# stablecabal/gyre

Hardware: AMD Instinct MI355X
Metric: SD1.5 512px 50-step images/sec (node) (higher is better)
Workload: dtype bf16

## Files before the change

gyre_amd/build.py:

```python
from __future__ import annotations

import os
import subprocess
import sys
from concurrent.futures import ThreadPoolExecutor

HERE = os.path.dirname(os.path.abspath(__file__))
CSRC = os.path.join(HERE, "csrc")
LIB = os.path.join(HERE, "libgyre_hip.so")
LIB_F16 = os.path.join(HERE, "libgyre_hip_f16.so")
SOURCES = ["kernels_elem.hip", "kernels_gemm.hip", "kernels_gemm4s.hip", "kernels_gemm_ar.hip", "kernels_gemm_sm.hip", "kernels_conv_out.hip", "kernels_attn.hip", "kernels_xattn.hip", "kernels_tome.hip", "kernels_bwd.hip", "kernels_t2i.hip", "model.hip", "model_vjp.hip", "model_t2i.hip"]
HEADERS = ["common.h", "kernels.h", "gemm_shared.h", "model_impl.h", os.path.join("..", "..", "include", "gyre_hip.h")]
FLAGS = ["--offload-arch=gfx950", "-O3", "-std=c++17", "-fPIC", "-mcode-object-version=5",
         "-Wno-unused-result", "-fno-gpu-rdc",
         "-mllvm", "-pragma-unroll-threshold=1000000"]


PER_FILE_FLAGS = {"kernels_attn.hip": ["-mllvm", "-amdgpu-mfma-vgpr-form=1"]}

RESOURCE_FILES = ("kernels_attn.hip", "kernels_gemm.hip", "kernels_gemm4s.hip", "kernels_gemm_ar.hip", "kernels_gemm_sm.hip")
SCRATCH_ALLOWED = ("k_attn3ILi80E", "k_gemm4s")
RESOURCES_JSON = os.path.join(HERE, "build", "kernel_resources.json")


def _hipcc() -> str:
    for c in (os.environ.get("HIPCC"), "/opt/rocm/bin/hipcc", "hipcc"):
        if c and (os.path.isabs(c) and os.path.exists(c) or not os.path.isabs(c)):
            return c
    raise RuntimeError("hipcc not found")


def _stale(out: str, deps) -> bool:
    if not os.path.exists(out):
        return True
    t = os.path.getmtime(out)
# ... 95 lines not shown
```

gyre_amd/csrc/kernels.h:

```cpp
#pragma once
#include "common.h"

int launch_nchw_to_nhwc(hipStream_t st, const void* x, int dtype, int B, int C, int HW, int Cpad, bf16_t* y);
int launch_add_nchw_into_nhwc(hipStream_t st, const void* r, int dtype, int B, int C, int HW, int Cpad, bf16_t* y);
int launch_ctx_to_bf16(hipStream_t st, const void* x, int dtype, size_t n, bf16_t* y);
int launch_dup_batch(hipStream_t st, const void* src, void* dst, size_t outer, size_t inner_bytes);
int launch_add_f32(hipStream_t st, float* y, const float* x, size_t n);
int launch_verify_hints(hipStream_t st, const int64_t* t, int B, int check_t, const void* x, size_t bytes_per_half, int check_pairs, int* flag);
int launch_timestep_embedding(hipStream_t st, const int64_t* t, int B, int dim, int flip, float shift, float* out);
int launch_rowvec_linear(hipStream_t st, float* x, int B, int K, const bf16_t* W, const float* bias, int N,
                         int act_in_silu, float* out, int ldo);
int launch_timestep_linear(hipStream_t st, const int64_t* t, int B, int dim, int flip, float shift, float* emb_scratch,
                           const bf16_t* W, const float* bias, int N, float* out, int ldo);

struct GnParams {
    const bf16_t* x; const bf16_t* x2; int C1;
    int B, HW, C, G;
    const float* gamma; const float* beta; float eps; int silu;
    float* partial;
    float* scale_shift;
    int nchunks;
    bf16_t* y;
    float* mean_rstd = nullptr;
    const float* cs_x = nullptr; int cs_x_chunks = 0;
// ... 15 lines not shown
    GEMM_DBG_NO_GN_FOLD       = 0x1000,
    GEMM_DBG_NO_XATTN         = 0x2000,
    GEMM_DBG_NO_GEGLU_4S      = 0x4000,
    GEMM_DBG_LN_STATS_PASS    = 0x8000,
    GEMM_DBG_GEGLU_NO_LN_FOLD = 0x10000,
    GEMM_DBG_GN_STATS_PASS    = 0x20000,
    GEMM_DBG_NO_128x160       = 0x40000,
    GEMM_DBG_NO_CS_128x160    = 0x100000,
    GEMM_DBG_NO_AR            = 0x200000,
    GEMM_DBG_AR_ALL           = 0x400000,
    GEMM_DBG_NO_4S_128_TILES  = 0x800000,
    GEMM_DBG_TWO_STAGE_LINEAR = 0x1000000,
    GEMM_DBG_DEEP_RING        = 0x2000000,
    GEMM_DBG_NO_W_BLOCK       = 0x4000000,
    GEMM_DBG_TWO_STAGE_CONV   = 0x8000000,
};
int launch_groupnorm_stats(hipStream_t st, const GnParams& p);
int launch_groupnorm_apply(hipStream_t st, const GnParams& p);
bool gn_use_small(int HW, int C, int C1, int G);
bool gn_accepts_colstats(const GnParams& p);
int launch_groupnorm_small(hipStream_t st, const GnParams& p);
int launch_gn_fold(hipStream_t st, const GnParams& p, const bf16_t* W, const float* bias, int N, bf16_t* Wf, float* bf);
int launch_layernorm(hipStream_t st, const bf16_t* x, int M, int C, const float* gamma, const float* beta, float eps,
                     bf16_t* y);
int launch_layernorm_stats(hipStream_t st, const bf16_t* x, int M, int C, float eps, float* stats);

int launch_nhwc_to_nchw_f32(hipStream_t st, const bf16_t* x, int B, int C, int HW, int Cpad, float* y);
int launch_repack_conv(hipStream_t st, const void* w, int dtype, int O, int I, int KH, int KW, int Ipad, bf16_t* out,
                       float scale = 1.f);
int launch_repack_linear(hipStream_t st, const void* w, int dtype, int O, int I, int geglu_interleave, bf16_t* out);
// ... 100 lines not shown
};
AttnPlan attn_plan(const AttnParams& p, int variant);
constexpr int ATTN_PLAN_INTS = 12, ATTN_BWD_PLAN_INTS = 10;
int launch_attention(hipStream_t st, const AttnParams& p);

struct XattnParams {
    const bf16_t* x; int ldx;
    const bf16_t* wq;
    const float* q_colsum; const float* q_bias;
    const float* ln_parts; int ln_nparts; const float* ln_stats; float ln_eps;
    const bf16_t* k; const bf16_t* vt; int ldvt;
    const bf16_t* wo; const float* bo;
    bf16_t* out; int ldo;
    float* rowstat_out;
    int M, rows_per_sample, Nk, heads;
};

bool xattn_supports(int C, int heads, int Nq, int Nk, int M);
int launch_xattn(hipStream_t st, const XattnParams& p, int C);

struct GnBwdParams {
    const bf16_t* x; const bf16_t* x2; int C1;
    int B, HW, C, G;
    const float* gamma; const float* beta; float eps; int silu;
    const bf16_t* dy;
    const bf16_t* addend;
    bf16_t* dx; bf16_t* dx2;
    float* partial = nullptr; const float* fwd_partial = nullptr; int nchunks = 0;
};
size_t gn_bwd_workspace_bytes(int B, int HW, int C, int G);
int launch_groupnorm_bwd(hipStream_t st, GnBwdParams p, void* ws);
int launch_layernorm_bwd(hipStream_t st, const bf16_t* x, const bf16_t* dy, int M, int C, const float* gamma, float eps,
                         const bf16_t* addend, bf16_t* dx);
int launch_geglu_bwd(hipStream_t st, const bf16_t* pre, const bf16_t* dy, size_t M, int F, bf16_t* dpre);
// ... 44 lines not shown
```

gyre_amd/csrc/kernels_xattn.hip:

```cpp
#include "gemm_shared.h"
#include <atomic>

namespace {
__device__ __forceinline__ void xa_dma16(unsigned dst, const void* src) {
    asm volatile("s_mov_b32 m0, %0\n\ts_nop 0\n\tglobal_load_lds_dwordx4 %1, off" ::"s"(dst), "v"(src) : "memory");
}
typedef __attribute__((ext_vector_type(4))) unsigned xa_u32x4;
}

template <int C, int D, int BM>
__global__ __launch_bounds__(512) void k_xattn(XattnParams p, unsigned long long* stamps) {
#define XA_STAMP(i_) do { if (stamps && threadIdx.x == 0) stamps[(size_t)blockIdx.x * 8 + (i_)] = __builtin_readcyclecounter(); } while (0)
    constexpr int H = C / D;
    constexpr int NH = 320, NP = C / NH;
    constexpr int WM = 2, WN = 4;
    constexpr int TM = BM / WM, TN = NH / WN, MI = TM / 16, NI = TN / 16;
    constexpr int ROWB = 2 * C, ROWS = ROWB / 16;
    constexpr int XO_BYTES = BM * ROWB, STAGE = NH * 128;
    constexpr int NKC = C / 64;
    constexpr int KSQ = (D + 31) / 32;
    constexpr int NKEY = 80, NKF = NKEY / 16;
    constexpr int DV = (D + 15) / 16;
    constexpr int KROW = DV * 32 + 16, VROW = NKEY * 2 + 16;
    constexpr int HEAD_BYTES = NKEY * KROW + DV * 16 * VROW;
    constexpr bool DBUF = 4 * HEAD_BYTES <= 2 * STAGE;
    constexpr int REGION = DBUF ? STAGE : 0;
    static_assert(C % NH == 0 && H == 8 && TM % 16 == 0 && TN % 16 == 0 && XO_BYTES + 2 * STAGE <= 160 * 1024 && 2 * HEAD_BYTES <= 2 * STAGE &&
                  (!DBUF || 2 * HEAD_BYTES <= STAGE), "tile / LDS budget");
    extern __shared__ __attribute__((aligned(16))) char smem[];
    char* xo = smem;
    char* ring = smem + XO_BYTES;
    const unsigned lds0 = (unsigned)(size_t)(__attribute__((address_space(3))) char*)smem;

    const int tid = threadIdx.x, lane = tid & 63;
    const int wave = __builtin_amdgcn_readfirstlane(tid >> 6);
    const int wm = wave / WN, wn = wave % WN;
    const int fr = lane & 15, fq = lane >> 4;
    const int m0 = blockIdx.x * BM;
    const int b = m0 / p.rows_per_sample;

    {
        constexpr int NT = XO_BYTES / 8192;
#pragma unroll
        for (int t = 0; t < NT; ++t) {
            const unsigned off = (unsigned)((t * 8 + wave) * 1024 + lane * 16);
            const unsigned row = off / ROWB, ps = (off - row * ROWB) >> 4;
            const unsigned ls = (ps & ~7u) | ((ps & 7u) ^ (row & 7u));
            xa_dma16(lds0 + (unsigned)((t * 8 + wave) * 1024), p.x + (size_t)(m0 + row) * p.ldx + ls * 8);
        }
    }
    XA_STAMP(0);
    const int r0 = tid >> 3;
    const int kvs = (tid & 7) ^ (r0 & 7);
    auto issue_w = [&](const bf16_t* W, int np, int kc, int slot) {
        const unsigned dst = lds0 + XO_BYTES + slot * STAGE + wave * 1024;
#pragma unroll
        for (int i = 0; i < NH / 64; ++i)
            xa_dma16(dst + i * 8192, W + (size_t)(np * NH + r0 + 64 * i) * C + kc * 64 + kvs * 8);
    };
    issue_w(p.wq, 0, 0, 0);

    float lrstd[MI], lrmu[MI];
    {
        const float invk = 1.0f / (float)C;
#pragma unroll
        for (int i = 0; i < MI; ++i) {
            const int m = m0 + wm * TM + i * 16 + fr;
            float2 rs;
            if (p.ln_nparts > 0) {
                float2 v[8];
#pragma unroll
                for (int t = 0; t < 8; ++t) if (t < p.ln_nparts) v[t] = ((const float2*)p.ln_parts)[(size_t)t * p.M + m];
                float su = 0.f, sq = 0.f;
#pragma unroll
                for (int t = 0; t < 8; ++t) if (t < p.ln_nparts) { su += v[t].x; sq += v[t].y; }
                for (int t = 8; t < p.ln_nparts; ++t) {
                    const float2 w2 = ((const float2*)p.ln_parts)[(size_t)t * p.M + m];
                    su += w2.x; sq += w2.y;
                }
                const float mean = su * invk;
                const float rstd = 1.0f / sqrtf(fmaxf(sq * invk - mean * mean, 0.f) + p.ln_eps);
                rs = make_float2(rstd, rstd * mean);
            } else {
                rs = ((const float2*)p.ln_stats)[m];
            }
            lrstd[i] = rs.x; lrmu[i] = rs.y;
        }
    }

    f32x4_t acc[MI][NI];
    auto projection = [&](const bf16_t* W, int first, auto&& pre, auto&& finish) {
        int slot = first;
        asm volatile("s_waitcnt vmcnt(0)" ::: "memory");
        __syncthreads();
#pragma unroll
        for (int np = 0; np < NP; ++np) {
#pragma unroll
            for (int i = 0; i < MI; ++i)
#pragma unroll
                for (int j = 0; j < NI; ++j) acc[i][j] = f32x4_t{0.f, 0.f, 0.f, 0.f};
            pre(np);
            for (int kc = 0; kc < NKC; ++kc) {
                if (kc + 1 < NKC) issue_w(W, np, kc + 1, slot ^ 1);
                else if (np + 1 < NP) issue_w(W, np + 1, 0, slot ^ 1);
                const uint4* a = (const uint4*)xo;
                const uint4* bw = (const uint4*)(ring + slot * STAGE);
#pragma unroll
                for (int ks = 0; ks < 2; ++ks) {
                    bf16x8_t af[MI];
#pragma unroll
                    for (int i = 0; i < MI; ++i) {
                        const int r = wm * TM + i * 16 + fr;
                        af[i] = __builtin_bit_cast(bf16x8_t, a[r * ROWS + kc * 8 + ((ks * 4 + fq) ^ (r & 7))]);
                    }
#pragma unroll
                    for (int j = 0; j < NI; ++j) {
                        const int r = wn * TN + j * 16 + fr;
                        const bf16x8_t bf = __builtin_bit_cast(bf16x8_t, bw[r * 8 + ((ks * 4 + fq) ^ (r & 7))]);
#pragma unroll
                        for (int i = 0; i < MI; ++i) acc[i][j] = GYRE_MFMA_16x16x32(bf, af[i], acc[i][j], 0, 0, 0);
                    }
                }
                asm volatile("s_waitcnt vmcnt(0) lgkmcnt(0)" ::: "memory");
                __syncthreads();
                slot ^= 1;
            }
            finish(np);
        }
    };
    auto xo_store4 = [&](int r, int n, uint2 v) {
        const int ls = n >> 3, ps = (ls & ~7) | ((ls & 7) ^ (r & 7));
        *(uint2*)(xo + r * ROWB + ps * 16 + (n & 7) * 2) = v;
    };
    uint2 pk[NP][MI][NI];
    auto flush_pk = [&]() {
#pragma unroll
        for (int np = 0; np < NP; ++np)
#pragma unroll
            for (int j = 0; j < NI; ++j)
#pragma unroll
                for (int i = 0; i < MI; ++i) xo_store4(wm * TM + i * 16 + fr, np * NH + wn * TN + j * 16 + 4 * fq, pk[np][i][j]);
    };

    XA_STAMP(1);
    float4 ccs[NI], cbb[NI];
    projection(p.wq, 0,
        [&](int np) {
#pragma unroll
            for (int j = 0; j < NI; ++j) {
                const int n = np * NH + wn * TN + j * 16 + 4 * fq;
                ccs[j] = *(const float4*)(p.q_colsum + n); cbb[j] = *(const float4*)(p.q_bias + n);
            }
        },
        [&](int np) {
#pragma unroll
            for (int j = 0; j < NI; ++j) {
                const float4 cs = ccs[j], bb = cbb[j];
#pragma unroll
                for (int i = 0; i < MI; ++i)
                    pk[np][i][j] = make_uint2(pack_bf16x2(fmaf(acc[i][j][0], lrstd[i], fmaf(-lrmu[i], cs.x, bb.x)), fmaf(acc[i][j][1], lrstd[i], fmaf(-lrmu[i], cs.y, bb.y))),
                                              pack_bf16x2(fmaf(acc[i][j][2], lrstd[i], fmaf(-lrmu[i], cs.z, bb.z)), fmaf(acc[i][j][3], lrstd[i], fmaf(-lrmu[i], cs.w, bb.w))));
            }
        });
    XA_STAMP(2);
    flush_pk();

    constexpr int RF = BM / 16, HG = 8 / RF;
    static_assert(RF * HG == 8 && (HG == 1 || HG == 2) && H % 2 == 0, "8 waves = row fragments x head groups");
    constexpr int KV = DV * 2;
    constexpr int VV = NKEY / 8;
    constexpr int NQK = (NKEY * KV + 511) / 512, NQV = (DV * 16 * VV + 511) / 512;
    const bf16_t* k_src[NQK]; int k_dst[NQK]; bool k_live[NQK], k_load[NQK];
// ... 38 lines not shown
    auto store_pair = [&](int pr) {
        char* base = ring + (pr & 1) * REGION;
#pragma unroll
        for (int e = 0; e < 2; ++e) {
#pragma unroll
            for (int q = 0; q < NQK; ++q)
                if (k_live[q]) *(xa_u32x4*)(base + e * HEAD_BYTES + k_dst[q]) = hk[e][q];
#pragma unroll
            for (int q = 0; q < NQV; ++q)
                if (v_live[q]) *(xa_u32x4*)(base + e * HEAD_BYTES + v_dst[q]) =
                    xa_u32x4{hv[e][q].x & vmask[q][0], hv[e][q].y & vmask[q][1], hv[e][q].z & vmask[q][2], hv[e][q].w & vmask[q][3]};
        }
    };
    const int qr = (wave % RF) * 16 + fr;
    const int hg = wave / RF;
    auto attend = [&](int h, const char* kb, const char* vb) {
        bf16x8_t qf[KSQ];
#pragma unroll
        for (int ks = 0; ks < KSQ; ++ks) {
            const int ls = (h * D + ks * 32 + fq * 8) >> 3;
            xa_u32x4 raw = {0u, 0u, 0u, 0u};
            if (ks * 32 + fq * 8 < D) raw = *(const xa_u32x4*)(xo + qr * ROWB + (((ls & ~7) | ((ls & 7) ^ (qr & 7))) << 4));
            qf[ks] = __builtin_bit_cast(bf16x8_t, raw);
        }
        f32x4_t s[NKF];
#pragma unroll
        for (int jk = 0; jk < NKF; ++jk) {
            s[jk] = f32x4_t{0.f, 0.f, 0.f, 0.f};
#pragma unroll
            for (int ks = 0; ks < KSQ; ++ks) {
                xa_u32x4 kraw = *(const xa_u32x4*)(kb + (jk * 16 + fr) * KROW + ks * 64 + fq * 16);
                if (ks * 32 + fq * 8 >= DV * 16) kraw = xa_u32x4{0u, 0u, 0u, 0u};
                s[jk] = GYRE_MFMA_16x16x32(__builtin_bit_cast(bf16x8_t, kraw), qf[ks], s[jk], 0, 0, 0);
            }
        }
        float mx = -1e30f;
#pragma unroll
        for (int jk = 0; jk < NKF; ++jk) {
            if ((jk + 1) * 16 > p.Nk) {
#pragma unroll
                for (int e = 0; e < 4; ++e)
                    if (jk * 16 + 4 * fq + e >= p.Nk) s[jk][e] = -1e30f;
            }
            mx = fmaxf(mx, fmaxf(fmaxf(s[jk][0], s[jk][1]), fmaxf(s[jk][2], s[jk][3])));
        }
        mx = fmaxf(mx, __shfl_xor(mx, 16));
        mx = fmaxf(mx, __shfl_xor(mx, 32));
        float l = 0.f;
#pragma unroll
        for (int jk = 0; jk < NKF; ++jk)
#pragma unroll
            for (int e = 0; e < 4; ++e) { s[jk][e] = __builtin_amdgcn_exp2f(s[jk][e] - mx); l += s[jk][e]; }
        l += __shfl_xor(l, 16);
        l += __shfl_xor(l, 32);
        f32x4_t o[DV];
#pragma unroll
        for (int di = 0; di < DV; ++di) o[di] = f32x4_t{0.f, 0.f, 0.f, 0.f};
#pragma unroll
        for (int t = 0; t < (NKF + 1) / 2; ++t) {
            constexpr int nkf_c = NKF;
            const bool second = 2 * t + 1 < nkf_c;
            const int t1 = second ? 2 * t + 1 : 0;
            xa_u32x4 pw;
            pw.x = pack_bf16x2(s[2 * t][0], s[2 * t][1]); pw.y = pack_bf16x2(s[2 * t][2], s[2 * t][3]);
            pw.z = second ? pack_bf16x2(s[t1][0], s[t1][1]) : 0u;
            pw.w = second ? pack_bf16x2(s[t1][2], s[t1][3]) : 0u;
            const bf16x8_t pf = __builtin_bit_cast(bf16x8_t, pw);
#pragma unroll
            for (int di = 0; di < DV; ++di) {
                const char* vrow = vb + (di * 16 + fr) * VROW + (32 * t + 4 * fq) * 2;
                const uint2 v0 = *(const uint2*)vrow;
                uint2 v1 = make_uint2(0u, 0u);
                if (second) v1 = *(const uint2*)(vrow + 32);
                const bf16x8_t vf = __builtin_bit_cast(bf16x8_t, xa_u32x4{v0.x, v0.y, v1.x, v1.y});
                o[di] = GYRE_MFMA_16x16x32(vf, pf, o[di], 0, 0, 0);
            }
        }
        const float inv = 1.0f / l;
#pragma unroll
        for (int di = 0; di < DV; ++di) {
            const int d = di * 16 + 4 * fq;
            if (d < D) xo_store4(qr, h * D + d, make_uint2(pack_bf16x2(o[di][0] * inv, o[di][1] * inv), pack_bf16x2(o[di][2] * inv, o[di][3] * inv)));
        }
    };
    fetch_pair(0);
    __syncthreads();
    XA_STAMP(3);
    uint2 res[NP][MI][NI];
#pragma unroll
    for (int np = 0; np < NP; ++np)
#pragma unroll
        for (int j = 0; j < NI; ++j) {
            const int n = np * NH + wn * TN + j * 16 + 4 * fq;
#pragma unroll
            for (int i = 0; i < MI; ++i) res[np][i][j] = *(const uint2*)(p.x + (size_t)(m0 + wm * TM + i * 16 + fr) * p.ldx + n);
        }
    store_pair(0);
    constexpr int NPAIR = H / 2;
    bool wo_requested = false;
    for (int pr = 0; pr < NPAIR; ++pr) {
        __syncthreads();
        if (pr + 1 < NPAIR) fetch_pair(pr + 1);
        else if (DBUF && (pr & 1) == 1) { issue_w(p.wo, 0, 0, 0); wo_requested = true; }
        const char* base = ring + (pr & 1) * REGION;
        if (HG == 1) {
            attend(2 * pr, base, base + NKEY * KROW);
            attend(2 * pr + 1, base + HEAD_BYTES, base + HEAD_BYTES + NKEY * KROW);
        } else {
            attend(2 * pr + hg, base + hg * HEAD_BYTES, base + hg * HEAD_BYTES + NKEY * KROW);
        }
        if (pr + 1 < NPAIR) {
            if (!DBUF) __syncthreads();
            store_pair(pr + 1);
        }
    }
    __syncthreads();

    XA_STAMP(4);
    if (!wo_requested) issue_w(p.wo, 0, 0, 0);
    projection(p.wo, 0,
        [&](int np) {
#pragma unroll
            for (int j = 0; j < NI; ++j)
                cbb[j] = p.bo ? *(const float4*)(p.bo + np * NH + wn * TN + j * 16 + 4 * fq) : make_float4(0.f, 0.f, 0.f, 0.f);
        },
        [&](int np) {
#pragma unroll
            for (int j = 0; j < NI; ++j) {
                const float4 bb = cbb[j];
#pragma unroll
                for (int i = 0; i < MI; ++i)
                    pk[np][i][j] = make_uint2(pack_bf16x2(acc[i][j][0] + bb.x + bf16lo(res[np][i][j].x), acc[i][j][1] + bb.y + bf16hi(res[np][i][j].x)),
                                              pack_bf16x2(acc[i][j][2] + bb.z + bf16lo(res[np][i][j].y), acc[i][j][3] + bb.w + bf16hi(res[np][i][j].y)));
            }
        });
    XA_STAMP(5);
    flush_pk();
    __syncthreads();
    for (int v = tid; v < BM * ROWS; v += 512) {
        const int r = v / ROWS, ls = v - r * ROWS;
        const int ps = (ls & ~7) | ((ls & 7) ^ (r & 7));
        *(uint4*)(p.out + (size_t)(m0 + r) * p.ldo + ls * 8) = *(const uint4*)(xo + r * ROWB + ps * 16);
    }
    XA_STAMP(6);
// ... 5 lines not shown
            for (int c = 0; c < VPL; ++c) {
                float f[8];
                unpack8(*(const uint4*)(xo + rr * ROWB + ((tid & 3) * VPL + c) * 16), f);
#pragma unroll
                for (int e = 0; e < 8; ++e) { su += f[e]; sq = fmaf(f[e], f[e], sq); }
            }
            su += __shfl_xor(su, 1); sq += __shfl_xor(sq, 1);
            su += __shfl_xor(su, 2); sq += __shfl_xor(sq, 2);
            if ((tid & 3) == 0) ((float2*)p.rowstat_out)[m0 + rr] = make_float2(su, sq);
        }
    }
    XA_STAMP(7);
#undef XA_STAMP
}

static thread_local unsigned long long* g_xattn_stamps = nullptr;
extern "C" int gyre_debug_xattn_stamps(void* dev_buf) { g_xattn_stamps = (unsigned long long*)dev_buf; return 0; }

bool xattn_supports(int C, int heads, int Nq, int Nk, int M) {
    if (heads != 8 || Nk < 1 || Nk > 80 || M <= 0) return false;
    if (C == 320) return Nq % 128 == 0 && M % 128 == 0 && M / 128 >= 256;
    return false;
}

template <int C, int D, int BM>
static int xattn_go(hipStream_t st, const XattnParams& p) {
    const int lds = 160 * 1024;
    auto kern = k_xattn<C, D, BM>;
    static std::atomic<unsigned long long> attr_done{0};
    if (gyre_lds_attr_needed(attr_done)) (void)hipFuncSetAttribute((const void*)kern, hipFuncAttributeMaxDynamicSharedMemorySize, lds);
    hipLaunchKernelGGL(kern, dim3(p.M / BM), dim3(512), lds, st, p, g_xattn_stamps);
    GYRE_LAUNCH_CHECK();
    return 0;
}

int launch_xattn(hipStream_t st, const XattnParams& p, int C) {
    if (!xattn_supports(C, p.heads, p.rows_per_sample, p.Nk, 256 * 128) || p.M <= 0 || p.M % 128)
        GYRE_FAIL(-6, "xattn: shape outside the fused cross-attention kernel's domain");
    if ((p.ldx % 8) || (p.ldo % 8) || (p.ldvt % 8) || ((((size_t)p.x | (size_t)p.out | (size_t)p.k | (size_t)p.vt | (size_t)p.wq | (size_t)p.wo) & 15) != 0))
        GYRE_FAIL(-1, "xattn: operands must be 16-byte aligned with strides that are multiples of 8 elements");
    const double fl = 2.0 * 2.0 * p.M * (double)C * C + 4.0 * p.M * (double)p.Nk * C;
    const double by = 3.0 * p.M * C * 2.0 + 2.0 * C * (double)C * 2.0;
    GyreProfScope prof_(KC_XATTN, st, fl, by);
    return xattn_go<320, 40, 128>(st, p);
}
```

gyre_amd/csrc/model.hip:

```cpp
#include "model_impl.h"

static thread_local std::string g_err;
static thread_local int64_t g_launches = 0;
void gyre_set_error(const std::string& msg) { g_err = msg; }
int64_t& gyre_launch_counter() { return g_launches; }
extern "C" const char* gyre_last_error(void) { return g_err.c_str(); }
extern "C" int gyre_abi_version(void) { return GYRE_ABI_VERSION; }
extern "C" int gyre_storage_dtype(void) { return GYRE_STORAGE_DTYPE; }
extern "C" int64_t gyre_last_launch_count(void) { return g_launches; }

namespace {
struct ProfRec { hipEvent_t a, b; int kclass; double flops, bytes; };
struct ProfState {
    unsigned long long mask = 0;
    std::vector<ProfRec> recs;
    std::vector<std::pair<hipEvent_t, hipEvent_t>> pool;
};
thread_local ProfState g_prof;
static_assert(KC_COUNT <= 64, "profiler mask is 64 bits wide");
}
GyreProfScope::GyreProfScope(int kclass, hipStream_t st, double flops, double bytes) : st_(st) {
    if (!(g_prof.mask >> kclass & 1ull)) return;
    hipEvent_t a, b;
    if (!g_prof.pool.empty()) { a = g_prof.pool.back().first; b = g_prof.pool.back().second; g_prof.pool.pop_back(); }
// ... 619 lines not shown
    if (!x || !gamma || !beta || !wq || !k || !vt || !wo || !ws || !out) GYRE_FAIL(GYRE_ERR_INVALID, "null argument");
    if (tokens <= 0 || M % tokens) GYRE_FAIL(GYRE_ERR_INVALID, "cross_attention_block: M must be a multiple of tokens");
    if (!xattn_supports(C, heads, tokens, Nk, M)) GYRE_FAIL(GYRE_ERR_UNSUPPORTED, "cross_attention_block: shape outside the fused kernel's domain");
    if (ws_bytes < gyre_op_ln_linear_workspace(C, C, M)) GYRE_FAIL(GYRE_ERR_WORKSPACE, "cross_attention_block: workspace too small");
    bf16_t* wf = (bf16_t*)ws;
    float* cs = (float*)((char*)ws + align_up((size_t)C * C * 2, 256));
    float* bb = (float*)((char*)cs + align_up((size_t)C * 4, 256));
    float* stats = (float*)((char*)bb + align_up((size_t)C * 4, 256));
    TRY(launch_ln_fold((hipStream_t)st, (const bf16_t*)wq, C, C, gamma, beta, nullptr, wf, cs, bb));
    TRY(launch_layernorm_stats((hipStream_t)st, (const bf16_t*)x, M, C, eps, stats));
    XattnParams xp;
    xp.x = (const bf16_t*)x; xp.ldx = C; xp.wq = wf; xp.q_colsum = cs; xp.q_bias = bb;
    xp.ln_parts = nullptr; xp.ln_nparts = 0; xp.ln_stats = stats; xp.ln_eps = eps;
    xp.k = (const bf16_t*)k; xp.vt = (const bf16_t*)vt; xp.ldvt = ldvt; xp.wo = (const bf16_t*)wo; xp.bo = bo;
    xp.out = (bf16_t*)out; xp.ldo = C; xp.rowstat_out = row_stats; xp.M = M; xp.rows_per_sample = tokens; xp.Nk = Nk; xp.heads = heads;
    return launch_xattn((hipStream_t)st, xp, C);
}
int gyre_op_nchw_to_nhwc(void* st, const void* x, int dtype, int B, int C, int HW, int Cpad, void* y) {
    if (!x || !y) GYRE_FAIL(GYRE_ERR_INVALID, "null argument");
    return launch_nchw_to_nhwc((hipStream_t)st, x, dtype, B, C, HW, Cpad, (bf16_t*)y);
}
int gyre_op_copy_probe(void* st, const void* src, void* dst, size_t bytes) {
    if (!src || !dst) GYRE_FAIL(GYRE_ERR_INVALID, "null argument");
    return launch_copy_probe((hipStream_t)st, src, dst, bytes);
}

}
```

gyre_amd/csrc/model_impl.h:

```cpp
#pragma once
#include "../../include/gyre_hip.h"
#include "kernels.h"
#include <cstdlib>
#include <cstdio>
#include <cmath>

#include <algorithm>
#include <array>
#include <cstring>
#include <map>
#include <memory>
#include <string>
#include <unordered_map>
#include <vector>

#define TRY(expr) do { int rc_ = (expr); if (rc_) return rc_; } while (0)
static inline size_t align_up(size_t v, size_t a) { return (v + a - 1) / a * a; }
static inline int pad8(int c) { return (c + 7) / 8 * 8; }

struct Arena {
    char* base = nullptr;
    size_t cap = 0, peak = 0;
    bool dry = false;
    std::map<size_t, size_t> free_;
// ... 76 lines not shown
        WtEntry& en = ar_cache[w];
        if (!en.p || en.bytes < bytes) {
            en.p = (bf16_t*)dmalloc(bytes, false);
            en.bytes = bytes; en.version = 0;
        }
        int& k = ar_kind[w];
        *fresh = en.p && en.version == weights_version && k == kind;
        if (en.p) { en.version = weights_version; k = kind; }
        return en.p;
    }
    std::unordered_map<const void*, WtEntry> blk_cache;
    bf16_t* blk_lookup(const void* w, size_t bytes, bool* fresh) {
        WtEntry& en = blk_cache[w];
        if (!en.p || en.bytes < bytes) {
            if (en.p) dfree(en.p);
            en.p = (bf16_t*)dmalloc(bytes, false);
            en.bytes = en.p ? bytes : 0; en.version = 0;
        }
        *fresh = en.p && en.version == weights_version;
        if (en.p) en.version = weights_version;
        return en.p;
    }
    void dfree(void* ptr) {
        for (size_t i = 0; i < allocs.size(); ++i)
            if (allocs[i] == ptr) { allocs[i] = allocs.back(); allocs.pop_back(); (void)hipDeviceSynchronize(); (void)hipFree(ptr); return; }
    }
    struct ScEntry { bf16_t* w = nullptr; float* b = nullptr; size_t elems = 0; uint64_t version = 0; };
    std::unordered_map<const void*, ScEntry> sc_cache;
    ScEntry* sc_lookup(const void* w, int N, int Kcat, bool* fresh) {
        ScEntry& en = sc_cache[w];
// ... 506 lines not shown
                        TRY(prep_blk(p, pf));
                        TRY(launch_gemm(st, p, pf));
                    }
                    free(stats);
                }
            }
            if (!fused) {
                TRY(normalise());
                TRY(linear(xq.p, C, nullptr, 0, 0, B * Nq, C, w.wqk, 2 * C, w.bqk, nullptr, 0, 0, q.p, 2 * C));
                TRY(linear_t(xq.p, C, B * Nq, C, w.wv, C, w.bv, Nq, ldvt, vt.p));
            }
            qp = q.p; kp = dry() ? nullptr : q.p + C; vtp = vt.p; ldq = ldk = 2 * C;
        } else {
            Nk = kv_rows_per_batch; ldvt = (Nk + 7) / 8 * 8;
            if (ln && !sv && ctx_cache && store && !w.bq && w.k_prescaled && residual.p == xq_in.p && !(gemm_planner_state() & GEMM_DBG_NO_XATTN) &&
                xattn_supports(C, w.heads, Nq, Nk, gemm_get_batch_invariant() > 0 ? gemm_get_batch_invariant() * Nq : B * Nq)) {
                if (ctx_layer >= ctx_cache->size()) GYRE_FAIL(GYRE_ERR_INVALID, "internal: context cache layer overflow");
                GemmParams pq;
                pq.A = xq_in.p; pq.lda = C; pq.mode = GEMM_LINEAR; pq.W = w.wq; pq.K = C; pq.N = C; pq.M = B * Nq; pq.bias = nullptr;
                Tn stats;
                TRY(ln_fold_into(pq, *ln, stats));
                TRY(alloc(out, B, xq.H, xq.W, C));
                if (rs_out) {
                    rs_out->nparts = 1;
                    TRY(alloc_raw(rs_out->t, (size_t)B * Nq * 2 * sizeof(float)));
                }
                if (!dry()) {
                    XattnParams xp;
                    xp.x = xq_in.p; xp.ldx = C; xp.wq = pq.W; xp.q_colsum = pq.ln_colsum; xp.q_bias = pq.bias;
                    xp.ln_parts = pq.ln_parts; xp.ln_nparts = pq.ln_nparts; xp.ln_stats = pq.ln_stats; xp.ln_eps = 1e-5f;
                    xp.k = (*ctx_cache)[ctx_layer].k; xp.vt = (*ctx_cache)[ctx_layer].vt; xp.ldvt = ldvt;
                    xp.wo = w.wo; xp.bo = w.bo; xp.out = out.p; xp.ldo = C;
                    xp.rowstat_out = rs_out ? (float*)rs_out->t.p : nullptr;
                    xp.M = B * Nq; xp.rows_per_sample = Nq; xp.Nk = Nk; xp.heads = w.heads;
                    TRY(launch_xattn(st, xp, C));
                }
                ++ctx_layer;
                free(stats);
                return 0;
            }
            TRY(alloc(q, B, xq.H, xq.W, C));
            if (ln) {
                TRY(ln_linear(xq_in, *ln, w.wq, C, w.bq, 0, q.p, C));
                ln = nullptr;
            } else {
                TRY(linear(xq.p, C, nullptr, 0, 0, B * Nq, C, w.wq, C, w.bq, nullptr, 0, 0, q.p, C));
            }
            if (ctx_cache) {
                if (ctx_layer >= ctx_cache->size()) GYRE_FAIL(GYRE_ERR_INVALID, "internal: context cache layer overflow");
// ... 720 lines not shown
```

Baseline: 8.824.

## Extend fused cross-attention kernel to C=640 with deeper weight ring and blocked weights

Extends the fused LN+Q-proj+cross-attention+O-proj kernel to the 640-channel UNet level, using a 4-stage ring of 64-byte weight rows and pre-blocked weight copies cached per weight. The goal is to cut the separate GEMM and attention launches and their intermediate HBM traffic at that resolution, and to get contiguous weight DMA. It also adds paired-head attention, preloaded column-sum and bias registers, and a hand-counted vmcnt wait scheme. The costs are extra cached device memory for the blocked weights, a lower 64-row tile, and fragile hand-set waitcnt values.

```diff
diff --git a/gyre_amd/build.py b/gyre_amd/build.py
--- a/gyre_amd/build.py
+++ b/gyre_amd/build.py
@@ -18,7 +18,7 @@
 
 PER_FILE_FLAGS = {"kernels_attn.hip": ["-mllvm", "-amdgpu-mfma-vgpr-form=1"]}
 
-RESOURCE_FILES = ("kernels_attn.hip", "kernels_gemm.hip", "kernels_gemm4s.hip", "kernels_gemm_ar.hip", "kernels_gemm_sm.hip")
+RESOURCE_FILES = ("kernels_attn.hip", "kernels_gemm.hip", "kernels_gemm4s.hip", "kernels_gemm_ar.hip", "kernels_gemm_sm.hip", "kernels_xattn.hip")
 SCRATCH_ALLOWED = ("k_attn3ILi80E", "k_gemm4s")
 RESOURCES_JSON = os.path.join(HERE, "build", "kernel_resources.json")
 
diff --git a/gyre_amd/csrc/kernels.h b/gyre_amd/csrc/kernels.h
--- a/gyre_amd/csrc/kernels.h
+++ b/gyre_amd/csrc/kernels.h
@@ -53,6 +53,7 @@
     GEMM_DBG_DEEP_RING        = 0x2000000,
     GEMM_DBG_NO_W_BLOCK       = 0x4000000,
     GEMM_DBG_TWO_STAGE_CONV   = 0x8000000,
+    GEMM_DBG_NO_XATTN_640     = 0x10000000,
 };
 int launch_groupnorm_stats(hipStream_t st, const GnParams& p);
 int launch_groupnorm_apply(hipStream_t st, const GnParams& p);
@@ -183,10 +184,13 @@
     bf16_t* out; int ldo;
     float* rowstat_out;
     int M, rows_per_sample, Nk, heads;
+    const bf16_t* wq_blk = nullptr; const bf16_t* wo_blk = nullptr;
 };
 
 bool xattn_supports(int C, int heads, int Nq, int Nk, int M);
 int launch_xattn(hipStream_t st, const XattnParams& p, int C);
+size_t xattn_wblock_bytes(int C);
+int launch_xattn_wblock(hipStream_t st, const bf16_t* W, int C, bf16_t* out);
 
 struct GnBwdParams {
     const bf16_t* x; const bf16_t* x2; int C1;
diff --git a/gyre_amd/csrc/kernels_xattn.hip b/gyre_amd/csrc/kernels_xattn.hip
--- a/gyre_amd/csrc/kernels_xattn.hip
+++ b/gyre_amd/csrc/kernels_xattn.hip
@@ -1,14 +1,20 @@
 #include "gemm_shared.h"
 #include <atomic>
+#include <type_traits>
+
+#ifndef XATTN_PAIRED
+#define XATTN_PAIRED 1
+#endif
 
 namespace {
 __device__ __forceinline__ void xa_dma16(unsigned dst, const void* src) {
     asm volatile("s_mov_b32 m0, %0\n\ts_nop 0\n\tglobal_load_lds_dwordx4 %1, off" ::"s"(dst), "v"(src) : "memory");
 }
 typedef __attribute__((ext_vector_type(4))) unsigned xa_u32x4;
-}
-
-template <int C, int D, int BM>
+template <typename T> __device__ __forceinline__ void xa_pin(T& v) { asm volatile("" : "+v"(v)); }
+}
+
+template <int C, int D, int BM, int NST, int KB>
 __global__ __launch_bounds__(512) void k_xattn(XattnParams p, unsigned long long* stamps) {
 #define XA_STAMP(i_) do { if (stamps && threadIdx.x == 0) stamps[(size_t)blockIdx.x * 8 + (i_)] = __builtin_readcyclecounter(); } while (0)
     constexpr int H = C / D;
@@ -16,17 +22,19 @@
     constexpr int WM = 2, WN = 4;
     constexpr int TM = BM / WM, TN = NH / WN, MI = TM / 16, NI = TN / 16;
     constexpr int ROWB = 2 * C, ROWS = ROWB / 16;
-    constexpr int XO_BYTES = BM * ROWB, STAGE = NH * 128;
-    constexpr int NKC = C / 64;
+    constexpr int RB = 2 * KB, SL = RB / 16;
+    constexpr int XO_BYTES = BM * ROWB, STAGE = NH * RB, RING = NST * STAGE;
+    constexpr int NKC = C / KB, T = NP * NKC;
     constexpr int KSQ = (D + 31) / 32;
     constexpr int NKEY = 80, NKF = NKEY / 16;
     constexpr int DV = (D + 15) / 16;
     constexpr int KROW = DV * 32 + 16, VROW = NKEY * 2 + 16;
     constexpr int HEAD_BYTES = NKEY * KROW + DV * 16 * VROW;
-    constexpr bool DBUF = 4 * HEAD_BYTES <= 2 * STAGE;
-    constexpr int REGION = DBUF ? STAGE : 0;
-    static_assert(C % NH == 0 && H == 8 && TM % 16 == 0 && TN % 16 == 0 && XO_BYTES + 2 * STAGE <= 160 * 1024 && 2 * HEAD_BYTES <= 2 * STAGE &&
-                  (!DBUF || 2 * HEAD_BYTES <= STAGE), "tile / LDS budget");
+    constexpr bool DBUF = 4 * HEAD_BYTES <= RING;
+    constexpr int REGION = DBUF ? RING / 2 : 0;
+    static_assert((NST == 2 && KB == 64) || (NST == 4 && KB == 32), "ring geometries built: 2 x 128-byte rows, 4 x 64-byte rows");
+    static_assert(C % NH == 0 && C % KB == 0 && H == 8 && TM % 16 == 0 && TN % 16 == 0 && XO_BYTES + RING <= 160 * 1024 && 2 * HEAD_BYTES <= RING &&
+                  (!DBUF || 2 * HEAD_BYTES <= REGION) && T >= NST, "tile / LDS budget");
     extern __shared__ __attribute__((aligned(16))) char smem[];
     char* xo = smem;
     char* ring = smem + XO_BYTES;
@@ -50,15 +58,42 @@
         }
     }
     XA_STAMP(0);
-    const int r0 = tid >> 3;
-    const int kvs = (tid & 7) ^ (r0 & 7);
-    auto issue_w = [&](const bf16_t* W, int np, int kc, int slot) {
-        const unsigned dst = lds0 + XO_BYTES + slot * STAGE + wave * 1024;
-#pragma unroll
-        for (int i = 0; i < NH / 64; ++i)
-            xa_dma16(dst + i * 8192, W + (size_t)(np * NH + r0 + 64 * i) * C + kc * 64 + kvs * 8);
-    };
-    issue_w(p.wq, 0, 0, 0);
+    const int wl = lane / SL;
+    const int wj = (wl >> 2) & 3;
+    const int fsw = SL == 8 ? (wl & 7) : ((((wj ^ (wj >> 1)) & 1) << 1) | (wj >> 1));
+    const int kvs = (lane % SL) ^ fsw;
+    constexpr int WI = STAGE / 1024, RPI = 1024 / RB;
+    auto issue_w = [&](const bf16_t* W, const bf16_t* Wb, int s) {
+        const int np = s / NKC, kc = s - np * NKC;
+        const unsigned dst = lds0 + XO_BYTES + (s % NST) * STAGE + wave * 1024;
+        const int rs = Wb ? KB : C;
+        const bf16_t* src = (Wb ? Wb + (size_t)s * NH * KB : W + (size_t)np * NH * C + kc * KB) + (size_t)(wave * RPI + wl) * rs + kvs * 8;
+#pragma unroll
+        for (int i = 0; i < (WI + 7) / 8; ++i)
+            if (8 * i + 8 <= WI || wave < WI - 8 * i) xa_dma16(dst + i * 8192, src + (size_t)(8 * RPI * i) * rs);
+    };
+    auto ring_wait = [&](int younger) {
+        if constexpr (NST == 2) {
+            asm volatile("s_waitcnt vmcnt(0) lgkmcnt(0)" ::: "memory");
+        } else {
+            static_assert(NST == 2 || WI == 20, "requests per wave and step: 3 / 2");
+            const bool big = wave < WI - 16;
+            if (younger >= 2) { if (big) asm volatile("s_waitcnt vmcnt(6) lgkmcnt(0)" ::: "memory"); else asm volatile("s_waitcnt vmcnt(4) lgkmcnt(0)" ::: "memory"); }
+            else if (younger == 1) { if (big) asm volatile("s_waitcnt vmcnt(3) lgkmcnt(0)" ::: "memory"); else asm volatile("s_waitcnt vmcnt(2) lgkmcnt(0)" ::: "memory"); }
+            else asm volatile("s_waitcnt vmcnt(0) lgkmcnt(0)" ::: "memory");
+        }
+    };
+#pragma unroll
+    for (int s = 0; s < NST - 1; ++s) issue_w(p.wq, p.wq_blk, s);
+
+    f32x4_t ccs[NP][NI], cbb[NP][NI];
+#pragma unroll
+    for (int np = 0; np < NP; ++np)
+#pragma unroll
+        for (int j = 0; j < NI; ++j) {
+            const int n = np * NH + wn * TN + j * 16 + 4 * fq;
+            ccs[np][j] = *(const f32x4_t*)(p.q_colsum + n); cbb[np][j] = *(const f32x4_t*)(p.q_bias + n);
+        }
 
     float lrstd[MI], lrmu[MI];
     {
@@ -89,44 +124,44 @@
     }
 
     f32x4_t acc[MI][NI];
-    auto projection = [&](const bf16_t* W, int first, auto&& pre, auto&& finish) {
-        int slot = first;
-        asm volatile("s_waitcnt vmcnt(0)" ::: "memory");
-        __syncthreads();
+    auto projection = [&](const bf16_t* W, const bf16_t* Wb, auto&& finish) {
+        int t = 0;
 #pragma unroll
         for (int np = 0; np < NP; ++np) {
 #pragma unroll
             for (int i = 0; i < MI; ++i)
 #pragma unroll
                 for (int j = 0; j < NI; ++j) acc[i][j] = f32x4_t{0.f, 0.f, 0.f, 0.f};
-            pre(np);
-            for (int kc = 0; kc < NKC; ++kc) {
-                if (kc + 1 < NKC) issue_w(W, np, kc + 1, slot ^ 1);
-                else if (np + 1 < NP) issue_w(W, np + 1, 0, slot ^ 1);
+            for (int kc = 0; kc < NKC; ++kc, ++t) {
+                ring_wait(min(NST - 2, T - 1 - t));
+                __builtin_amdgcn_s_barrier();
+                if (t + NST - 1 < T) issue_w(W, Wb, t + NST - 1);
                 const uint4* a = (const uint4*)xo;
-                const uint4* bw = (const uint4*)(ring + slot * STAGE);
-#pragma unroll
-                for (int ks = 0; ks < 2; ++ks) {
+                const uint4* bw = (const uint4*)(ring + (t % NST) * STAGE);
+#pragma unroll
+                for (int ks = 0; ks < KB / 32; ++ks) {
+                    const int ls = kc * (KB / 8) + ks * 4 + fq;
                     bf16x8_t af[MI];
 #pragma unroll
                     for (int i = 0; i < MI; ++i) {
                         const int r = wm * TM + i * 16 + fr;
-                        af[i] = __builtin_bit_cast(bf16x8_t, a[r * ROWS + kc * 8 + ((ks * 4 + fq) ^ (r & 7))]);
+                        af[i] = __builtin_bit_cast(bf16x8_t, a[r * ROWS + ((ls & ~7) | ((ls & 7) ^ (r & 7)))]);
                     }
 #pragma unroll
                     for (int j = 0; j < NI; ++j) {
                         const int r = wn * TN + j * 16 + fr;
-                        const bf16x8_t bf = __builtin_bit_cast(bf16x8_t, bw[r * 8 + ((ks * 4 + fq) ^ (r & 7))]);
+                        const int fj = (fr >> 2) & 3;
+                        const int sw = SL == 8 ? (r & 7) : ((((fj ^ (fj >> 1)) & 1) << 1) | (fj >> 1));
+                        const bf16x8_t bf = __builtin_bit_cast(bf16x8_t, bw[r * SL + ((ks * 4 + fq) ^ sw)]);
 #pragma unroll
                         for (int i = 0; i < MI; ++i) acc[i][j] = GYRE_MFMA_16x16x32(bf, af[i], acc[i][j], 0, 0, 0);
                     }
                 }
-                asm volatile("s_waitcnt vmcnt(0) lgkmcnt(0)" ::: "memory");
-                __syncthreads();
-                slot ^= 1;
             }
             finish(np);
         }
+        asm volatile("s_waitcnt lgkmcnt(0)" ::: "memory");
+        __builtin_amdgcn_s_barrier();
     };
     auto xo_store4 = [&](int r, int n, uint2 v) {
         const int ls = n >> 3, ps = (ls & ~7) | ((ls & 7) ^ (r & 7));
@@ -143,19 +178,17 @@
     };
 
     XA_STAMP(1);
-    float4 ccs[NI], cbb[NI];
-    projection(p.wq, 0,
+#pragma unroll
+    for (int np = 0; np < NP; ++np)
+#pragma unroll
+        for (int j = 0; j < NI; ++j) { xa_pin(ccs[np][j]); xa_pin(cbb[np][j]); }
+#pragma unroll
+    for (int i = 0; i < MI; ++i) { xa_pin(lrstd[i]); xa_pin(lrmu[i]); }
+    projection(p.wq, p.wq_blk,
         [&](int np) {
 #pragma unroll
             for (int j = 0; j < NI; ++j) {
-                const int n = np * NH + wn * TN + j * 16 + 4 * fq;
-                ccs[j] = *(const float4*)(p.q_colsum + n); cbb[j] = *(const float4*)(p.q_bias + n);
-            }
-        },
-        [&](int np) {
-#pragma unroll
-            for (int j = 0; j < NI; ++j) {
-                const float4 cs = ccs[j], bb = cbb[j];
+                const f32x4_t cs = ccs[np][j], bb = cbb[np][j];
 #pragma unroll
                 for (int i = 0; i < MI; ++i)
                     pk[np][i][j] = make_uint2(pack_bf16x2(fmaf(acc[i][j][0], lrstd[i], fmaf(-lrmu[i], cs.x, bb.x)), fmaf(acc[i][j][1], lrstd[i], fmaf(-lrmu[i], cs.y, bb.y))),
@@ -224,73 +257,98 @@
     };
     const int qr = (wave % RF) * 16 + fr;
     const int hg = wave / RF;
-    auto attend = [&](int h, const char* kb, const char* vb) {
-        bf16x8_t qf[KSQ];
-#pragma unroll
-        for (int ks = 0; ks < KSQ; ++ks) {
-            const int ls = (h * D + ks * 32 + fq * 8) >> 3;
-            xa_u32x4 raw = {0u, 0u, 0u, 0u};
-            if (ks * 32 + fq * 8 < D) raw = *(const xa_u32x4*)(xo + qr * ROWB + (((ls & ~7) | ((ls & 7) ^ (qr & 7))) << 4));
-            qf[ks] = __builtin_bit_cast(bf16x8_t, raw);
-        }
-        f32x4_t s[NKF];
-#pragma unroll
-        for (int jk = 0; jk < NKF; ++jk) {
-            s[jk] = f32x4_t{0.f, 0.f, 0.f, 0.f};
-#pragma unroll
-            for (int ks = 0; ks < KSQ; ++ks) {
-                xa_u32x4 kraw = *(const xa_u32x4*)(kb + (jk * 16 + fr) * KROW + ks * 64 + fq * 16);
-                if (ks * 32 + fq * 8 >= DV * 16) kraw = xa_u32x4{0u, 0u, 0u, 0u};
-                s[jk] = GYRE_MFMA_16x16x32(__builtin_bit_cast(bf16x8_t, kraw), qf[ks], s[jk], 0, 0, 0);
-            }
-        }
-        float mx = -1e30f;
+    auto attend = [&](auto ne_c, int h0, const char* kb, const char* vb) {
+        constexpr int NE = decltype(ne_c)::value;
+        bf16x8_t qf[NE][KSQ];
+#pragma unroll
+        for (int ks = 0; ks < KSQ; ++ks)
+#pragma unroll
+            for (int e = 0; e < NE; ++e) {
+                const int ls = ((h0 + e) * D + ks * 32 + fq * 8) >> 3;
+                xa_u32x4 raw = {0u, 0u, 0u, 0u};
+                if (ks * 32 + fq * 8 < D) raw = *(const xa_u32x4*)(xo + qr * ROWB + (((ls & ~7) | ((ls & 7) ^ (qr & 7))) << 4));
+                qf[e][ks] = __builtin_bit_cast(bf16x8_t, raw);
+            }
+        f32x4_t s[NE][NKF];
+#pragma unroll
+        for (int jk = 0; jk < NKF; ++jk)
+#pragma unroll
+            for (int e = 0; e < NE; ++e) {
+                s[e][jk] = f32x4_t{0.f, 0.f, 0.f, 0.f};
+#pragma unroll
+                for (int ks = 0; ks < KSQ; ++ks) {
+                    xa_u32x4 kraw = *(const xa_u32x4*)(kb + e * HEAD_BYTES + (jk * 16 + fr) * KROW + ks * 64 + fq * 16);
+                    if (ks * 32 + fq * 8 >= DV * 16) kraw = xa_u32x4{0u, 0u, 0u, 0u};
+                    s[e][jk] = GYRE_MFMA_16x16x32(__builtin_bit_cast(bf16x8_t, kraw), qf[e][ks], s[e][jk], 0, 0, 0);
+                }
+            }
+        float mx[NE], l[NE];
+#pragma unroll
+        for (int e = 0; e < NE; ++e) mx[e] = -1e30f;
 #pragma unroll
         for (int jk = 0; jk < NKF; ++jk) {
             if ((jk + 1) * 16 > p.Nk) {
 #pragma unroll
-                for (int e = 0; e < 4; ++e)
-                    if (jk * 16 + 4 * fq + e >= p.Nk) s[jk][e] = -1e30f;
-            }
-            mx = fmaxf(mx, fmaxf(fmaxf(s[jk][0], s[jk][1]), fmaxf(s[jk][2], s[jk][3])));
-        }
-        mx = fmaxf(mx, __shfl_xor(mx, 16));
-        mx = fmaxf(mx, __shfl_xor(mx, 32));
-        float l = 0.f;
-#pragma unroll
-        for (int jk = 0; jk < NKF; ++jk)
-#pragma unroll
-            for (int e = 0; e < 4; ++e) { s[jk][e] = __builtin_amdgcn_exp2f(s[jk][e] - mx); l += s[jk][e]; }
-        l += __shfl_xor(l, 16);
-        l += __shfl_xor(l, 32);
-        f32x4_t o[DV];
-#pragma unroll
-        for (int di = 0; di < DV; ++di) o[di] = f32x4_t{0.f, 0.f, 0.f, 0.f};
+                for (int e = 0; e < NE; ++e)
+#pragma unroll
+                    for (int c = 0; c < 4; ++c)
+                        if (jk * 16 + 4 * fq + c >= p.Nk) s[e][jk][c] = -1e30f;
+            }
+#pragma unroll
+            for (int e = 0; e < NE; ++e) mx[e] = fmaxf(mx[e], fmaxf(fmaxf(s[e][jk][0], s[e][jk][1]), fmaxf(s[e][jk][2], s[e][jk][3])));
+        }
+#pragma unroll
+        for (int e = 0; e < NE; ++e) mx[e] = fmaxf(mx[e], __shfl_xor(mx[e], 16));
+#pragma unroll
+        for (int e = 0; e < NE; ++e) mx[e] = fmaxf(mx[e], __shfl_xor(mx[e], 32));
+#pragma unroll
+        for (int e = 0; e < NE; ++e) {
+            l[e] = 0.f;
+#pragma unroll
+            for (int jk = 0; jk < NKF; ++jk)
+#pragma unroll
+                for (int c = 0; c < 4; ++c) { s[e][jk][c] = __builtin_amdgcn_exp2f(s[e][jk][c] - mx[e]); l[e] += s[e][jk][c]; }
+        }
+#pragma unroll
+        for (int e = 0; e < NE; ++e) l[e] += __shfl_xor(l[e], 16);
+#pragma unroll
+        for (int e = 0; e < NE; ++e) l[e] += __shfl_xor(l[e], 32);
+        f32x4_t o[NE][DV];
+#pragma unroll
+        for (int e = 0; e < NE; ++e)
+#pragma unroll
+            for (int di = 0; di < DV; ++di) o[e][di] = f32x4_t{0.f, 0.f, 0.f, 0.f};
 #pragma unroll
         for (int t = 0; t < (NKF + 1) / 2; ++t) {
             constexpr int nkf_c = NKF;
             const bool second = 2 * t + 1 < nkf_c;
             const int t1 = second ? 2 * t + 1 : 0;
-            xa_u32x4 pw;
-            pw.x = pack_bf16x2(s[2 * t][0], s[2 * t][1]); pw.y = pack_bf16x2(s[2 * t][2], s[2 * t][3]);
-            pw.z = second ? pack_bf16x2(s[t1][0], s[t1][1]) : 0u;
-            pw.w = second ? pack_bf16x2(s[t1][2], s[t1][3]) : 0u;
-            const bf16x8_t pf = __builtin_bit_cast(bf16x8_t, pw);
+#pragma unroll
+            for (int e = 0; e < NE; ++e) {
+                xa_u32x4 pw;
+                pw.x = pack_bf16x2(s[e][2 * t][0], s[e][2 * t][1]); pw.y = pack_bf16x2(s[e][2 * t][2], s[e][2 * t][3]);
+                pw.z = second ? pack_bf16x2(s[e][t1][0], s[e][t1][1]) : 0u;
+                pw.w = second ? pack_bf16x2(s[e][t1][2], s[e][t1][3]) : 0u;
+                const bf16x8_t pf = __builtin_bit_cast(bf16x8_t, pw);
+#pragma unroll
+                for (int di = 0; di < DV; ++di) {
+                    const char* vrow = vb + e * HEAD_BYTES + (di * 16 + fr) * VROW + (32 * t + 4 * fq) * 2;
+                    const uint2 v0 = *(const uint2*)vrow;
+                    uint2 v1 = make_uint2(0u, 0u);
+                    if (second) v1 = *(const uint2*)(vrow + 32);
+                    const bf16x8_t vf = __builtin_bit_cast(bf16x8_t, xa_u32x4{v0.x, v0.y, v1.x, v1.y});
+                    o[e][di] = GYRE_MFMA_16x16x32(vf, pf, o[e][di], 0, 0, 0);
+                }
+            }
+        }
+#pragma unroll
+        for (int e = 0; e < NE; ++e) {
+            const float inv = 1.0f / l[e];
 #pragma unroll
             for (int di = 0; di < DV; ++di) {
-                const char* vrow = vb + (di * 16 + fr) * VROW + (32 * t + 4 * fq) * 2;
-                const uint2 v0 = *(const uint2*)vrow;
-                uint2 v1 = make_uint2(0u, 0u);
-                if (second) v1 = *(const uint2*)(vrow + 32);
-                const bf16x8_t vf = __builtin_bit_cast(bf16x8_t, xa_u32x4{v0.x, v0.y, v1.x, v1.y});
-                o[di] = GYRE_MFMA_16x16x32(vf, pf, o[di], 0, 0, 0);
-            }
-        }
-        const float inv = 1.0f / l;
-#pragma unroll
-        for (int di = 0; di < DV; ++di) {
-            const int d = di * 16 + 4 * fq;
-            if (d < D) xo_store4(qr, h * D + d, make_uint2(pack_bf16x2(o[di][0] * inv, o[di][1] * inv), pack_bf16x2(o[di][2] * inv, o[di][3] * inv)));
+                const int d = di * 16 + 4 * fq;
+                if (d < D) xo_store4(qr, (h0 + e) * D + d, make_uint2(pack_bf16x2(o[e][di][0] * inv, o[e][di][1] * inv), pack_bf16x2(o[e][di][2] * inv, o[e][di][3] * inv)));
+            }
         }
     };
     fetch_pair(0);
@@ -304,6 +362,7 @@
             const int n = np * NH + wn * TN + j * 16 + 4 * fq;
 #pragma unroll
             for (int i = 0; i < MI; ++i) res[np][i][j] = *(const uint2*)(p.x + (size_t)(m0 + wm * TM + i * 16 + fr) * p.ldx + n);
+            cbb[np][j] = p.bo ? *(const f32x4_t*)(p.bo + n) : f32x4_t{0.f, 0.f, 0.f, 0.f};
         }
     store_pair(0);
     constexpr int NPAIR = H / 2;
@@ -311,13 +370,17 @@
     for (int pr = 0; pr < NPAIR; ++pr) {
         __syncthreads();
         if (pr + 1 < NPAIR) fetch_pair(pr + 1);
-        else if (DBUF && (pr & 1) == 1) { issue_w(p.wo, 0, 0, 0); wo_requested = true; }
+        else if (DBUF && (pr & 1) == 1) { issue_w(p.wo, p.wo_blk, 0); wo_requested = true; }
         const char* base = ring + (pr & 1) * REGION;
         if (HG == 1) {
-            attend(2 * pr, base, base + NKEY * KROW);
-            attend(2 * pr + 1, base + HEAD_BYTES, base + HEAD_BYTES + NKEY * KROW);
+#if XATTN_PAIRED
+            attend(std::integral_constant<int, 2>{}, 2 * pr, base, base + NKEY * KROW);
+#else
+            attend(std::integral_constant<int, 1>{}, 2 * pr, base, base + NKEY * KROW);
+            attend(std::integral_constant<int, 1>{}, 2 * pr + 1, base + HEAD_BYTES, base + HEAD_BYTES + NKEY * KROW);
+#endif
         } else {
-            attend(2 * pr + hg, base + hg * HEAD_BYTES, base + hg * HEAD_BYTES + NKEY * KROW);
+            attend(std::integral_constant<int, 1>{}, 2 * pr + hg, base + hg * HEAD_BYTES, base + hg * HEAD_BYTES + NKEY * KROW);
         }
         if (pr + 1 < NPAIR) {
             if (!DBUF) __syncthreads();
@@ -327,17 +390,22 @@
     __syncthreads();
 
     XA_STAMP(4);
-    if (!wo_requested) issue_w(p.wo, 0, 0, 0);
-    projection(p.wo, 0,
+#pragma unroll
+    for (int np = 0; np < NP; ++np)
+#pragma unroll
+        for (int j = 0; j < NI; ++j) {
+            xa_pin(cbb[np][j]);
+#pragma unroll
+            for (int i = 0; i < MI; ++i) { xa_pin(res[np][i][j].x); xa_pin(res[np][i][j].y); }
+        }
+    if (!wo_requested) issue_w(p.wo, p.wo_blk, 0);
+#pragma unroll
+    for (int s = 1; s < NST - 1; ++s) issue_w(p.wo, p.wo_blk, s);
+    projection(p.wo, p.wo_blk,
         [&](int np) {
 #pragma unroll
-            for (int j = 0; j < NI; ++j)
-                cbb[j] = p.bo ? *(const float4*)(p.bo + np * NH + wn * TN + j * 16 + 4 * fq) : make_float4(0.f, 0.f, 0.f, 0.f);
-        },
-        [&](int np) {
-#pragma unroll
             for (int j = 0; j < NI; ++j) {
-                const float4 bb = cbb[j];
+                const f32x4_t bb = cbb[np][j];
 #pragma unroll
                 for (int i = 0; i < MI; ++i)
                     pk[np][i][j] = make_uint2(pack_bf16x2(acc[i][j][0] + bb.x + bf16lo(res[np][i][j].x), acc[i][j][1] + bb.y + bf16hi(res[np][i][j].x)),
@@ -373,19 +441,41 @@
 #undef XA_STAMP
 }
 
+__global__ void k_xattn_wblock(const bf16_t* __restrict__ W, int C, bf16_t* __restrict__ out) {
+    const int v = blockIdx.x * blockDim.x + threadIdx.x;
+    if (v >= C * C / 8) return;
+    const int q = v & 3, r = (v >> 2) % 320, s = (v >> 2) / 320, nkc = C / 32;
+    const int np = s / nkc, kc = s - np * nkc;
+    ((uint4*)out)[v] = *(const uint4*)(W + (size_t)(np * 320 + r) * C + kc * 32 + q * 8);
+}
+#ifndef XATTN_WBLOCK
+#define XATTN_WBLOCK 1
+#endif
+size_t xattn_wblock_bytes(int C) { return XATTN_WBLOCK && C == 640 ? (size_t)C * C * 2 : 0; }
+int launch_xattn_wblock(hipStream_t st, const bf16_t* W, int C, bf16_t* out) {
+    if (!xattn_wblock_bytes(C) || !W || !out || (((size_t)W | (size_t)out) & 15)) GYRE_FAIL(-1, "xattn: no blocked weight form for this shape");
+    hipLaunchKernelGGL(k_xattn_wblock, dim3((C * C / 8 + 255) / 256), dim3(256), 0, st, W, C, out);
+    GYRE_LAUNCH_CHECK();
+    return 0;
+}
+
+#ifndef XATTN_C320_NST
+#define XATTN_C320_NST 2
+#endif
 static thread_local unsigned long long* g_xattn_stamps = nullptr;
 extern "C" int gyre_debug_xattn_stamps(void* dev_buf) { g_xattn_stamps = (unsigned long long*)dev_buf; return 0; }
 
 bool xattn_supports(int C, int heads, int Nq, int Nk, int M) {
     if (heads != 8 || Nk < 1 || Nk > 80 || M <= 0) return false;
     if (C == 320) return Nq % 128 == 0 && M % 128 == 0 && M / 128 >= 256;
+    if (C == 640) return Nq % 64 == 0 && M % 64 == 0 && M / 64 >= 256;
     return false;
 }
 
-template <int C, int D, int BM>
+template <int C, int D, int BM, int NST, int KB>
 static int xattn_go(hipStream_t st, const XattnParams& p) {
     const int lds = 160 * 1024;
-    auto kern = k_xattn<C, D, BM>;
+    auto kern = k_xattn<C, D, BM, NST, KB>;
     static std::atomic<unsigned long long> attr_done{0};
     if (gyre_lds_attr_needed(attr_done)) (void)hipFuncSetAttribute((const void*)kern, hipFuncAttributeMaxDynamicSharedMemorySize, lds);
     hipLaunchKernelGGL(kern, dim3(p.M / BM), dim3(512), lds, st, p, g_xattn_stamps);
@@ -394,12 +484,15 @@
 }
 
 int launch_xattn(hipStream_t st, const XattnParams& p, int C) {
-    if (!xattn_supports(C, p.heads, p.rows_per_sample, p.Nk, 256 * 128) || p.M <= 0 || p.M % 128)
+    const int BM = C == 640 ? 64 : 128;
+    if (!xattn_supports(C, p.heads, p.rows_per_sample, p.Nk, 256 * BM) || p.M <= 0 || p.M % BM)
         GYRE_FAIL(-6, "xattn: shape outside the fused cross-attention kernel's domain");
     if ((p.ldx % 8) || (p.ldo % 8) || (p.ldvt % 8) || ((((size_t)p.x | (size_t)p.out | (size_t)p.k | (size_t)p.vt | (size_t)p.wq | (size_t)p.wo) & 15) != 0))
         GYRE_FAIL(-1, "xattn: operands must be 16-byte aligned with strides that are multiples of 8 elements");
     const double fl = 2.0 * 2.0 * p.M * (double)C * C + 4.0 * p.M * (double)p.Nk * C;
     const double by = 3.0 * p.M * C * 2.0 + 2.0 * C * (double)C * 2.0;
     GyreProfScope prof_(KC_XATTN, st, fl, by);
-    return xattn_go<320, 40, 128>(st, p);
-}
+    if (C == 640) return xattn_go<640, 80, 64, 4, 32>(st, p);
+    if (p.wq_blk || p.wo_blk) GYRE_FAIL(-1, "xattn: blocked weight copies belong to the C = 640 form");
+    return xattn_go<320, 40, 128, XATTN_C320_NST, XATTN_C320_NST == 4 ? 32 : 64>(st, p);
+}
diff --git a/gyre_amd/csrc/model.hip b/gyre_amd/csrc/model.hip
--- a/gyre_amd/csrc/model.hip
+++ b/gyre_amd/csrc/model.hip
@@ -657,6 +657,14 @@
     xp.ln_parts = nullptr; xp.ln_nparts = 0; xp.ln_stats = stats; xp.ln_eps = eps;
     xp.k = (const bf16_t*)k; xp.vt = (const bf16_t*)vt; xp.ldvt = ldvt; xp.wo = (const bf16_t*)wo; xp.bo = bo;
     xp.out = (bf16_t*)out; xp.ldo = C; xp.rowstat_out = row_stats; xp.M = M; xp.rows_per_sample = tokens; xp.Nk = Nk; xp.heads = heads;
+    const size_t base = align_up(gyre_op_ln_linear_workspace(C, C, M), 256), wb = xattn_wblock_bytes(C);
+    if (wb && ws_bytes >= base + 2 * wb) {
+        bf16_t* qb = (bf16_t*)((char*)ws + base);
+        bf16_t* ob = (bf16_t*)((char*)ws + base + wb);
+        TRY(launch_xattn_wblock((hipStream_t)st, wf, C, qb));
+        TRY(launch_xattn_wblock((hipStream_t)st, (const bf16_t*)wo, C, ob));
+        xp.wq_blk = qb; xp.wo_blk = ob;
+    }
     return launch_xattn((hipStream_t)st, xp, C);
 }
 int gyre_op_nchw_to_nhwc(void* st, const void* x, int dtype, int B, int C, int HW, int Cpad, void* y) {
diff --git a/gyre_amd/csrc/model_impl.h b/gyre_amd/csrc/model_impl.h
--- a/gyre_amd/csrc/model_impl.h
+++ b/gyre_amd/csrc/model_impl.h
@@ -114,6 +114,17 @@
         WtEntry& en = blk_cache[w];
         if (!en.p || en.bytes < bytes) {
             if (en.p) dfree(en.p);
+            en.p = (bf16_t*)dmalloc(bytes, false);
+            en.bytes = en.p ? bytes : 0; en.version = 0;
+        }
+        *fresh = en.p && en.version == weights_version;
+        if (en.p) en.version = weights_version;
+        return en.p;
+    }
+    std::unordered_map<const void*, WtEntry> xblk_cache;
+    bf16_t* xblk_lookup(const void* w, size_t bytes, bool* fresh) {
+        WtEntry& en = xblk_cache[w];
+        if (!en.p || en.bytes < bytes) {
             en.p = (bf16_t*)dmalloc(bytes, false);
             en.bytes = en.p ? bytes : 0; en.version = 0;
         }
@@ -650,6 +661,7 @@
         } else {
             Nk = kv_rows_per_batch; ldvt = (Nk + 7) / 8 * 8;
             if (ln && !sv && ctx_cache && store && !w.bq && w.k_prescaled && residual.p == xq_in.p && !(gemm_planner_state() & GEMM_DBG_NO_XATTN) &&
+                !(C == 640 && (gemm_planner_state() & GEMM_DBG_NO_XATTN_640)) &&
                 xattn_supports(C, w.heads, Nq, Nk, gemm_get_batch_invariant() > 0 ? gemm_get_batch_invariant() * Nq : B * Nq)) {
                 if (ctx_layer >= ctx_cache->size()) GYRE_FAIL(GYRE_ERR_INVALID, "internal: context cache layer overflow");
                 GemmParams pq;
@@ -669,6 +681,18 @@
                     xp.wo = w.wo; xp.bo = w.bo; xp.out = out.p; xp.ldo = C;
                     xp.rowstat_out = rs_out ? (float*)rs_out->t.p : nullptr;
                     xp.M = B * Nq; xp.rows_per_sample = Nq; xp.Nk = Nk; xp.heads = w.heads;
+                    if (const size_t bb = xattn_wblock_bytes(C)) {
+                        const bf16_t* src[2] = {xp.wq, xp.wo};
+                        const bf16_t* blk[2] = {nullptr, nullptr};
+                        for (int i = 0; i < 2; ++i) {
+                            bool fresh = false;
+                            bf16_t* b_ = store->xblk_lookup(src[i], bb, &fresh);
+                            if (!b_) { (void)hipGetLastError(); continue; }
+                            if (!fresh) TRY(launch_xattn_wblock(st, src[i], C, b_));
+                            blk[i] = b_;
+                        }
+                        xp.wq_blk = blk[0]; xp.wo_blk = blk[1];
+                    }
                     TRY(launch_xattn(st, xp, C));
                 }
                 ++ctx_layer;
```

Measured after the change: 8.834 (median of 3 runs). No clear change (+0.1%).
